# reazon-research/ReazonSpeech

Measured on AMD Instinct MI355X. Metric: RTFx (audio-sec/wall-sec), FastConformer-RNNT 619M batch=256, higher is better.
Workload: dtype bf16

## Files before the change

reazonspeech_amd/csrc/k_rnnt.hip:

```cpp
#include <cstdio>
#include <cstdlib>

#include "k_rnnt_common.h"

namespace {

__global__ void rnnt_init_kernel(DecodeState st, const int32_t* __restrict__ enc_lens, int B, int blank,
                                 int32_t* __restrict__ n_ids) {
    __shared__ int n_alive_s;
    if (threadIdx.x == 0) n_alive_s = 0;
    __syncthreads();
    for (int b = threadIdx.x; b < B; b += blockDim.x) {
        st.tcur[b] = 0; st.sym[b] = 0; st.token[b] = blank; st.act[b] = b;
        if (st.token2) st.token2[b] = -1;
        n_ids[b] = 0;
        if (enc_lens[b] > 0) st.alive[atomicAdd(&n_alive_s, 1)] = b;
    }
    __syncthreads();
    if (threadIdx.x == 0) { st.counters[0] = B; st.counters[1] = 0; st.counters[2] = n_alive_s; st.counters[3] = 0; }
}

__global__ __launch_bounds__(1024) void rnnt_lstm_kernel(DecodeState st, int layer, int B, int H,
                                                        const float* __restrict__ embed,
                                                        const float* __restrict__ W ,
                                                        const float* __restrict__ bias ) {
    extern __shared__ __attribute__((aligned(16))) char lstm_smem[];
    float (*part)[4][32][16] = reinterpret_cast<float (*)[4][32][16]>(lstm_smem);
    int* rows_s = reinterpret_cast<int*>(lstm_smem + SPLITK_LSTM * 4 * 32 * 16 * 4);
    const int n_act = st.counters[0];
    const int rt = blockIdx.y, ut = blockIdx.x;
    if (rt * 32 >= n_act) return;
    const int tid = threadIdx.x, lane = tid & 63, wave = tid >> 6;
    if (tid < 32) {
        const int i = rt * 32 + tid;
        rows_s[tid] = st.act[i < n_act ? i : n_act - 1];
    }
    __syncthreads();
    const int li = lane & 15, kk = lane >> 4;
    const int lr = lane >> 2, lc = lane & 3;
    const int perm = 4 * (4 * li + kk);
    const int K = 2 * H, kslice = K / SPLITK_LSTM, nkb = K / 16;
    const float* xsrc[2];
    const float* hsrc[2];
#pragma unroll
    for (int ri = 0; ri < 2; ++ri) {
        const int row = rows_s[ri * 16 + lr];
        xsrc[ri] = layer == 0 ? embed + (size_t)st.token[row] * H : st.h_tmp + ((size_t)(layer - 1) * B + row) * H;
        hsrc[ri] = st.h + ((size_t)layer * B + row) * H;
    }
    const float* wfrag[4];
#pragma unroll
    for (int gt = 0; gt < 4; ++gt) wfrag[gt] = W + ((size_t)((gt * H) / 16 + ut) * nkb) * 256 + lane * 4;
    f32x4_t acc[2][4];
#pragma unroll
    for (int ri = 0; ri < 2; ++ri)
#pragma unroll
        for (int gt = 0; gt < 4; ++gt) acc[ri][gt] = (f32x4_t){0.f, 0.f, 0.f, 0.f};
    struct Frag { float4 a[2], w[4]; };
    auto load = [&](int k0) {
        Frag fr;
        const int k = k0 + 4 * lc;
#pragma unroll
        for (int ri = 0; ri < 2; ++ri)
            fr.a[ri] = (k < H) ? *reinterpret_cast<const float4*>(xsrc[ri] + k)
                               : *reinterpret_cast<const float4*>(hsrc[ri] + (k - H));
#pragma unroll
        for (int gt = 0; gt < 4; ++gt) fr.w[gt] = *reinterpret_cast<const float4*>(wfrag[gt] + (size_t)(k0 >> 4) * 256);
        return fr;
    };
    auto compute = [&](const Frag& fin) {
        Frag fr = fin;
#pragma unroll
        for (int ri = 0; ri < 2; ++ri) fr.a[ri] = to_mfma_a_layout(fin.a[ri], perm);
#define RS_MFMA_E(c)                                                                                            \
        _Pragma("unroll") for (int ri = 0; ri < 2; ++ri) _Pragma("unroll") for (int gt = 0; gt < 4; ++gt)      \
            acc[ri][gt] = __builtin_amdgcn_mfma_f32_16x16x4f32(fr.a[ri].c, fr.w[gt].c, acc[ri][gt], 0, 0, 0);
        RS_MFMA_E(x) RS_MFMA_E(y) RS_MFMA_E(z) RS_MFMA_E(w)
#undef RS_MFMA_E
    };
    const int kbeg = wave * kslice, nblk = kslice / 16;
    {
        Frag f0 = load(kbeg);
        Frag f1 = nblk > 1 ? load(kbeg + 16) : f0;
        int u = 0;
        for (; u + 2 < nblk; ++u) {
            const Frag f2 = load(kbeg + 16 * (u + 2));
            compute(f0);
            f0 = f1;
            f1 = f2;
        }
        if (nblk >= 2) { compute(f0); f0 = f1; }
        compute(f0);
    }
#pragma unroll
    for (int ri = 0; ri < 2; ++ri)
#pragma unroll
        for (int gt = 0; gt < 4; ++gt)
#pragma unroll
            for (int r = 0; r < 4; ++r) part[wave][gt][ri * 16 + 4 * kk + r][li] = acc[ri][gt][r];
    __syncthreads();
    if (tid >= 512) return;
    const int i = tid >> 4, j = tid & 15;
    if (rt * 32 + i >= n_act) return;
    const int brow = rows_s[i];
    const int unit = ut * 16 + j;
    float z[4];
#pragma unroll
    for (int gt = 0; gt < 4; ++gt) {
        float s = part[0][gt][i][j];
#pragma unroll
        for (int sl = 1; sl < SPLITK_LSTM; ++sl) s = s + part[sl][gt][i][j];
        z[gt] = s + bias[gt * H + unit];
    }
    const float ig = rs_sigmoidf(z[0]), fg = rs_sigmoidf(z[1]), gg = rs_tanhf(z[2]), og = rs_sigmoidf(z[3]);
    const size_t o = ((size_t)layer * B + brow) * H + unit;
    const float cn = fmaf(fg, st.c[o], ig * gg);
    st.c_tmp[o] = cn;
    st.h_tmp[o] = og * rs_tanhf(cn);
}

template <int MODE>
__global__ __launch_bounds__(512) void rnnt_tile_kernel(DecodeState st, const float* __restrict__ f, int B, int Tp,
                                                        int L, int H, int K, int N, const float* __restrict__ W,
                                                        const float* __restrict__ bias, int n_ctiles, int step,
                                                        int rows_per_utt) {
    extern __shared__ __attribute__((aligned(16))) char tile_smem[];
    float (*part)[32][65] = reinterpret_cast<float (*)[32][65]>(tile_smem);
    int* rows_s = reinterpret_cast<int*>(tile_smem + SPLITK_TILE * 32 * 65 * 4);
    int rt = blockIdx.y;
    const int ct = blockIdx.x;
    const int tid = threadIdx.x, lane = tid & 63, wave = tid >> 6;
    constexpr bool WALK = MODE == 3 || MODE == 4;
    constexpr bool ARGMAX = MODE == 1 || MODE == 5;
    const int32_t* list = MODE == 0 ? st.act : st.alive + (size_t)(step & 1) * B;
    const int la = MODE == 5 ? rows_per_utt : 1;
    const int n_rows = MODE == 0 ? st.counters[0] : st.counters[2 + (step & 1)] * la;
    if (MODE >= 1 && rt == 0 && ct == 0 && tid == 0) {
        st.counters[0] = 0;
        st.counters[2 + ((step + 1) & 1)] = 0;
    }
    if (MODE >= 1 && ct >= n_ctiles) return;
    for (;; rt += gridDim.y) {
    if (rt * 32 >= n_rows) return;
    if (tid < 32) {
        int i = rt * 32 + tid;
        i = i < n_rows ? i : n_rows - 1;
        rows_s[tid] = MODE == 5 ? list[i / la] * la + i % la : list[i];
    }
    __syncthreads();
    const int li = lane & 15, kk = lane >> 4;
    const int lr = lane >> 2, lc = lane & 3;
    const int perm = 4 * (4 * li + kk);
    const float* asrc[2];
    const float* gsrc[2];
#pragma unroll
    for (int ri = 0; ri < 2; ++ri) {
        const int row = rows_s[ri * 16 + lr];
        if (MODE == 0) {
            asrc[ri] = st.h_tmp + ((size_t)(L - 1) * B + row) * H;
            gsrc[ri] = nullptr;
        } else {
            if (MODE == 4) {
                asrc[ri] = st.a_pre + (size_t)row * K;
                gsrc[ri] = nullptr;
            } else if (MODE == 5) {
                const int utt = row / la;
                int t = st.tcur[utt] + row % la;
                t = t < Tp ? t : Tp - 1;
                asrc[ri] = f + ((size_t)utt * Tp + t) * K;
                gsrc[ri] = st.g + (size_t)utt * K;
            } else {
                int t = st.tcur[row];
                t = t < Tp ? t : Tp - 1;
                const int utt = MODE >= 2 ? row / rows_per_utt : row;
                asrc[ri] = f + ((size_t)utt * Tp + t) * K;
                gsrc[ri] = MODE == 3 ? st.g + st.g_off[row] : st.g + (size_t)row * K;
            }
        }
    }
    const int nkb = K / 16, ntile = (N + 15) / 16;
    const float* wfrag[4];
#pragma unroll
    for (int cj = 0; cj < 4; ++cj) {
        int tn = ct * 4 + cj;
        tn = tn < ntile ? tn : ntile - 1;
        wfrag[cj] = W + ((size_t)tn * nkb) * 256 + lane * 4;
    }
    f32x4_t acc[2][4];
#pragma unroll
    for (int ri = 0; ri < 2; ++ri)
#pragma unroll
        for (int cj = 0; cj < 4; ++cj) acc[ri][cj] = (f32x4_t){0.f, 0.f, 0.f, 0.f};
    constexpr bool HAS_G = (MODE >= 1 && MODE <= 3) || MODE == 5;
    struct Frag { float4 a[2], g[2], w[4]; };
    auto load = [&](int k0) {
        Frag fr;
        const int k = k0 + 4 * lc;
#pragma unroll
        for (int ri = 0; ri < 2; ++ri) {
            fr.a[ri] = *reinterpret_cast<const float4*>(asrc[ri] + k);
            if (HAS_G) fr.g[ri] = *reinterpret_cast<const float4*>(gsrc[ri] + k);
        }
#pragma unroll
        for (int cj = 0; cj < 4; ++cj) fr.w[cj] = *reinterpret_cast<const float4*>(wfrag[cj] + (size_t)(k0 >> 4) * 256);
        return fr;
    };
    auto compute = [&](const Frag& fr) {
        float4 a[2];
#pragma unroll
        for (int ri = 0; ri < 2; ++ri) {
            a[ri] = fr.a[ri];
            if (HAS_G) {
                if (st.joint_act) {
                    a[ri].x = rs_tanhf(a[ri].x + fr.g[ri].x); a[ri].y = rs_tanhf(a[ri].y + fr.g[ri].y);
                    a[ri].z = rs_tanhf(a[ri].z + fr.g[ri].z); a[ri].w = rs_tanhf(a[ri].w + fr.g[ri].w);
// ... 94 lines not shown
        const int oi = st.pidx[(size_t)b * n_ctiles + ctile];
        if (ov > val || (ov == val && oi < idx)) { val = ov; idx = oi; }
    }
#pragma unroll
    for (int off = 32; off > 0; off >>= 1) {
        const float ov = __shfl_xor(val, off, 64);
        const int oi = __shfl_xor(idx, off, 64);
        if (ov > val || (ov == val && oi < idx)) { val = ov; idx = oi; }
    }
    if (lane != 0) return;
    int t = st.tcur[b], sy = st.sym[b];
    bool emitted = false;
    if (idx == blank || idx == st.unk || idx == 0x7fffffff) {
        t += 1; sy = 0;
    } else {
        const int n = n_ids[b];
        if (n < u_max) { ids[(size_t)b * u_max + n] = idx; frames[(size_t)b * u_max + n] = t; n_ids[b] = n + 1; }
        else st.counters[1] = 1;
        if (st.token2) st.token2[b] = st.token[b];
        st.token[b] = idx;
        emitted = true;
        sy += 1;
        if (sy >= max_symbols) { t += 1; sy = 0; }
    }
    st.tcur[b] = t; st.sym[b] = sy;
    if (t < enc_lens[b]) {
        const int pos = atomicAdd(&st.counters[2 + ((step + 1) & 1)], 1);
        st.alive[(size_t)((step + 1) & 1) * B + pos] = b;
        if (emitted) { const int pa = atomicAdd(&st.counters[0], 1); st.act[pa] = b; }
    }
}



__global__ __launch_bounds__(256) void rnnt_finalize_la_kernel(DecodeState st, const int32_t* __restrict__ enc_lens, int B, int n_ctiles,
                                                               int blank, int max_symbols, int u_max, int step, int la,
                                                               int32_t* __restrict__ ids, int32_t* __restrict__ frames,
                                                               int32_t* __restrict__ n_ids) {
    const int lane = threadIdx.x & 63;
    const int slot = blockIdx.x * 4 + (threadIdx.x >> 6);
    const int n_alive = st.counters[2 + (step & 1)];
    if (slot >= n_alive) return;
    const int b = st.alive[(size_t)(step & 1) * B + slot];
    const int T = enc_lens[b];
    int t = st.tcur[b], sy = st.sym[b];
    bool emitted = false;
    for (int j = 0; j < la && t < T; ++j) {
        float val = -INFINITY;
        int idx = 0x7fffffff;
        const size_t row = (size_t)b * la + j;
        for (int ctile = lane; ctile < n_ctiles; ctile += 64) {
            const float ov = st.pmax[row * n_ctiles + ctile];
            const int oi = st.pidx[row * n_ctiles + ctile];
            if (ov > val || (ov == val && oi < idx)) { val = ov; idx = oi; }
        }
#pragma unroll
        for (int off = 32; off > 0; off >>= 1) {
            const float ov = __shfl_xor(val, off, 64);
            const int oi = __shfl_xor(idx, off, 64);
            if (ov > val || (ov == val && oi < idx)) { val = ov; idx = oi; }
        }
        if (idx == blank || idx == st.unk || idx == 0x7fffffff) { t += 1; sy = 0; continue; }
        if (lane == 0) {
            const int n = n_ids[b];
            if (n < u_max) { ids[(size_t)b * u_max + n] = idx; frames[(size_t)b * u_max + n] = t; n_ids[b] = n + 1; }
            else st.counters[1] = 1;
            if (st.token2) st.token2[b] = st.token[b];
            st.token[b] = idx;
        }
        emitted = true;
        sy += 1;
        if (sy >= max_symbols) { t += 1; sy = 0; }
        break;
    }
    if (lane != 0) return;
    st.tcur[b] = t; st.sym[b] = sy;
    if (t < T) {
        const int pos = atomicAdd(&st.counters[2 + ((step + 1) & 1)], 1);
        st.alive[(size_t)((step + 1) & 1) * B + pos] = b;
        if (emitted) { const int pa = atomicAdd(&st.counters[0], 1); st.act[pa] = b; }
    }
}

__global__ __launch_bounds__(1024) void rnnt_lstm4_kernel(DecodeState st, int layer, int B, int H,
                                                         const float* __restrict__ embed,
                                                         const float* __restrict__ W4 ,
                                                         const float* __restrict__ bias ) {
    __shared__ float part[SPLITK_LSTM][32][17];
    __shared__ int rows_s[32];
    const int n_act = st.counters[0];
    const int rt = blockIdx.y, ug = blockIdx.x;
    if (rt * 32 >= n_act) return;
    const int tid = threadIdx.x, lane = tid & 63, wave = tid >> 6;
    if (tid < 32) {
        const int i = rt * 32 + tid;
        rows_s[tid] = st.act[i < n_act ? i : n_act - 1];
    }
    __syncthreads();
    const int li = lane & 15, kk = lane >> 4;
    const int lr = lane >> 2, lc = lane & 3;
    const int perm = 4 * (4 * li + kk);
    const int K = 2 * H, kslice = K / SPLITK_LSTM, nkb = K / 16;
    const float* xsrc[2];
    const float* hsrc[2];
#pragma unroll
    for (int ri = 0; ri < 2; ++ri) {
        const int row = rows_s[ri * 16 + lr];
        xsrc[ri] = layer == 0 ? embed + (size_t)st.token[row] * H : st.h_tmp + ((size_t)(layer - 1) * B + row) * H;
        hsrc[ri] = st.h + ((size_t)layer * B + row) * H;
    }
    const float* wfrag = W4 + ((size_t)ug * nkb) * 256 + lane * 4;
    f32x4_t acc[2] = {(f32x4_t){0.f, 0.f, 0.f, 0.f}, (f32x4_t){0.f, 0.f, 0.f, 0.f}};
    const int kbeg = wave * kslice, nblk = kslice / 16;
    float4 av[2][8], wv[8];
#pragma unroll
    for (int u = 0; u < 8; ++u)
        if (u < nblk) {
            const int k = kbeg + 16 * u + 4 * lc;
#pragma unroll
            for (int ri = 0; ri < 2; ++ri)
                av[ri][u] = (k < H) ? *reinterpret_cast<const float4*>(xsrc[ri] + k) : *reinterpret_cast<const float4*>(hsrc[ri] + (k - H));
            wv[u] = *reinterpret_cast<const float4*>(wfrag + (size_t)((kbeg >> 4) + u) * 256);
        }
#pragma unroll
    for (int u = 0; u < 8; ++u)
        if (u < nblk) {
            const float4 a0 = to_mfma_a_layout(av[0][u], perm), a1 = to_mfma_a_layout(av[1][u], perm);
#define RS_MFMA_E(c)                                                                         \
            acc[0] = __builtin_amdgcn_mfma_f32_16x16x4f32(a0.c, wv[u].c, acc[0], 0, 0, 0);   \
            acc[1] = __builtin_amdgcn_mfma_f32_16x16x4f32(a1.c, wv[u].c, acc[1], 0, 0, 0);
            RS_MFMA_E(x) RS_MFMA_E(y) RS_MFMA_E(z) RS_MFMA_E(w)
#undef RS_MFMA_E
        }
#pragma unroll
    for (int ri = 0; ri < 2; ++ri)
#pragma unroll
        for (int r = 0; r < 4; ++r) part[wave][ri * 16 + 4 * kk + r][li] = acc[ri][r];
    __syncthreads();
    if (tid >= 128) return;
    const int i = tid >> 2, u4 = tid & 3;
    if (rt * 32 + i >= n_act) return;
    const int brow = rows_s[i];
    const int unit = ug * 4 + u4;
    float z[4];
#pragma unroll
    for (int gt = 0; gt < 4; ++gt) {
        float sm = part[0][i][gt * 4 + u4];
#pragma unroll
        for (int sl = 1; sl < SPLITK_LSTM; ++sl) sm = sm + part[sl][i][gt * 4 + u4];
        z[gt] = sm + bias[gt * H + unit];
    }
    const float ig = rs_sigmoidf(z[0]), fg = rs_sigmoidf(z[1]), gg = rs_tanhf(z[2]), og = rs_sigmoidf(z[3]);
    const size_t o = ((size_t)layer * B + brow) * H + unit;
    const float cn = fmaf(fg, st.c[o], ig * gg);
    st.c_tmp[o] = cn;
    st.h_tmp[o] = og * rs_tanhf(cn);
}

__global__ __launch_bounds__(512) void rnnt_pred16_kernel(DecodeState st, int B, int L, int H, int N ,
                                                         const float* __restrict__ W, const float* __restrict__ bias) {
    __shared__ float part[SPLITK_TILE][32][17];
    __shared__ int rows_s[32];
    const int rt = blockIdx.y, ct = blockIdx.x;
    const int tid = threadIdx.x, lane = tid & 63, wave = tid >> 6;
    const int n_rows = st.counters[0];
    if (rt * 32 >= n_rows) return;
    if (tid < 32) {
        const int i = rt * 32 + tid;
        rows_s[tid] = st.act[i < n_rows ? i : n_rows - 1];
    }
    __syncthreads();
    const int li = lane & 15, kk = lane >> 4;
    const int lr = lane >> 2, lc = lane & 3;
    const int perm = 4 * (4 * li + kk);
    const int K = H, nkb = K / 16;
    const float* asrc[2];
#pragma unroll
    for (int ri = 0; ri < 2; ++ri) asrc[ri] = st.h_tmp + ((size_t)(L - 1) * B + rows_s[ri * 16 + lr]) * H;
    const float* wfrag = W + ((size_t)ct * nkb) * 256 + lane * 4;
    f32x4_t acc[2] = {(f32x4_t){0.f, 0.f, 0.f, 0.f}, (f32x4_t){0.f, 0.f, 0.f, 0.f}};
    const int kslice = K / SPLITK_TILE, kbeg = wave * kslice, nblk = kslice / 16;
    float4 av[2][8], wv[8];
#pragma unroll
    for (int u = 0; u < 8; ++u)
        if (u < nblk) {
            const int k = kbeg + 16 * u + 4 * lc;
#pragma unroll
            for (int ri = 0; ri < 2; ++ri) av[ri][u] = *reinterpret_cast<const float4*>(asrc[ri] + k);
            wv[u] = *reinterpret_cast<const float4*>(wfrag + (size_t)((kbeg >> 4) + u) * 256);
        }
#pragma unroll
    for (int u = 0; u < 8; ++u)
        if (u < nblk) {
            const float4 a0 = to_mfma_a_layout(av[0][u], perm), a1 = to_mfma_a_layout(av[1][u], perm);
#define RS_MFMA_E(c)                                                                         \
            acc[0] = __builtin_amdgcn_mfma_f32_16x16x4f32(a0.c, wv[u].c, acc[0], 0, 0, 0);   \
            acc[1] = __builtin_amdgcn_mfma_f32_16x16x4f32(a1.c, wv[u].c, acc[1], 0, 0, 0);
            RS_MFMA_E(x) RS_MFMA_E(y) RS_MFMA_E(z) RS_MFMA_E(w)
#undef RS_MFMA_E
        }
#pragma unroll
    for (int ri = 0; ri < 2; ++ri)
#pragma unroll
        for (int r = 0; r < 4; ++r) part[wave][ri * 16 + 4 * kk + r][li] = acc[ri][r];
    __syncthreads();
    const int i = tid >> 4, c = tid & 15;
    const bool row_ok = rt * 32 + i < n_rows;
    const int brow = rows_s[i];
    const int v = ct * 16 + c;
    if (row_ok && v < N) {
        float sm = part[0][i][c];
#pragma unroll
        for (int sl = 1; sl < SPLITK_TILE; ++sl) sm = sm + part[sl][i][c];
        st.g[(size_t)brow * N + v] = sm + bias[v];
    }
    if (row_ok) {
        const int nct = gridDim.x;
        for (int l = 0; l < L; ++l)
            for (int u = ct * 16 + c; u < H; u += nct * 16) {
                const size_t o = ((size_t)l * B + brow) * H + u;
                st.h[o] = st.h_tmp[o];
                st.c[o] = st.c_tmp[o];
            }
    }
}

__global__ __launch_bounds__(256) void rnnt_prep_kernel(DecodeState st, const float* __restrict__ f, int B, int Tp, int J,
                                                        int step) {
    const int lane = threadIdx.x & 63;
    const int slot = blockIdx.x * 4 + (threadIdx.x >> 6);
    if (blockIdx.x == 0 && threadIdx.x == 0) {
        st.counters[0] = 0;
        st.counters[2 + ((step + 1) & 1)] = 0;
    }
    if (slot >= st.counters[2 + (step & 1)]) return;
    const int b = st.alive[(size_t)(step & 1) * B + slot];
    int t = st.tcur[b];
    t = t < Tp ? t : Tp - 1;
    const float* fr = f + ((size_t)b * Tp + t) * J;
    const float* gr = st.g + (size_t)b * J;
    float ss = 0.0f;
    for (int k = 4 * lane; k < J; k += 256) {
        const float4 fv = *reinterpret_cast<const float4*>(fr + k), gv = *reinterpret_cast<const float4*>(gr + k);
        float a0, a1, a2, a3;
        if (st.joint_act) {
            a0 = rs_tanhf(fv.x + gv.x); a1 = rs_tanhf(fv.y + gv.y); a2 = rs_tanhf(fv.z + gv.z); a3 = rs_tanhf(fv.w + gv.w);
        } else {
            a0 = fmaxf(fv.x + gv.x, 0.0f); a1 = fmaxf(fv.y + gv.y, 0.0f); a2 = fmaxf(fv.z + gv.z, 0.0f); a3 = fmaxf(fv.w + gv.w, 0.0f);
        }
        ss = fmaf(a0, a0, fmaf(a1, a1, fmaf(a2, a2, fmaf(a3, a3, ss))));
        *reinterpret_cast<u16x4_t*>(st.a16 + (size_t)slot * J + k) = pack_bf16x4(a0, a1, a2, a3);
    }
    ss = wave_sum(ss);
    if (lane == 0) st.anorm[slot] = sqrtf(ss) * 1.0001f + 0x1p-55f;
}

__global__ __launch_bounds__(256) void rnnt_screen_kernel(DecodeState st, const float* __restrict__ f, int B, int Tp, int J,
                                                          int Vpad, const uint16_t* __restrict__ W16,
                                                          const float* __restrict__ bpad, int step) {
    extern __shared__ __attribute__((aligned(16))) char scr_smem[];
    const int ldrow = J * 2 + 16;
    const int ct = blockIdx.x, rt = blockIdx.y;
    const int tid = threadIdx.x, lane = tid & 63, wave = tid >> 6;
    const int n_alive = st.counters[2 + (step & 1)];
    if (rt * 32 >= n_alive) return;
    const int col0 = (ct * 4 + wave) * 16;
    const bool has_cols = col0 < Vpad;
    const int li = lane & 15, kc = lane >> 4;
    const int nks = J / 32;
    const uint16_t* wrow = W16 + (size_t)((has_cols ? col0 : 0) + li) * J + kc * 8;
    bf16x8_t wf[20];
#pragma unroll
    for (int q = 0; q < 20; ++q)
        if (q < nks) wf[q] = *reinterpret_cast<const bf16x8_t*>(wrow + q * 32);
    const float bv = bpad[(has_cols ? col0 : 0) + li];
    {
        const int per_row = J / 8;
        for (int idx = tid; idx < 32 * per_row; idx += 256) {
            const int r = idx / per_row, c = idx - r * per_row;
            const int i = rt * 32 + r;
            const uint4 v = *reinterpret_cast<const uint4*>(st.a16 + (size_t)(i < n_alive ? i : n_alive - 1) * J + c * 8);
            *reinterpret_cast<uint4*>(scr_smem + r * ldrow + c * 16) = v;
        }
    }
    __syncthreads();
    if (!has_cols) return;
    f32x4_t acc[2] = {(f32x4_t){0.f, 0.f, 0.f, 0.f}, (f32x4_t){0.f, 0.f, 0.f, 0.f}};
#pragma unroll
    for (int q = 0; q < 20; ++q)
        if (q < nks) {
#pragma unroll
            for (int ri = 0; ri < 2; ++ri) {
                const bf16x8_t af = *reinterpret_cast<const bf16x8_t*>(scr_smem + (ri * 16 + li) * ldrow + (q * 32 + kc * 8) * 2);
                acc[ri] = __builtin_amdgcn_mfma_f32_16x16x32_bf16(af, wf[q], acc[ri], 0, 0, 0);
            }
        }
#pragma unroll
    for (int ri = 0; ri < 2; ++ri)
#pragma unroll
        for (int r = 0; r < 4; ++r) {
            const int slot = rt * 32 + ri * 16 + 4 * kc + r;
            if (slot < n_alive) st.zapprox[(size_t)slot * Vpad + col0 + li] = acc[ri][r] + bv;
        }
}

__device__ __forceinline__ float screen_margin(float m, float wmax, float anorm) {
// ... 167 lines not shown
    float zr[NCHW];
#pragma unroll
    for (int c = 0; c < NCHW; ++c) {
        const int col = (wave * NCHW + c) * 64 + lane;
        zr[c] = col < V ? z[col] : -INFINITY;
    }
    float m = -INFINITY;
#pragma unroll
    for (int c = 0; c < NCHW; ++c) m = fmaxf(m, zr[c]);
    m = wave_max(m);
    float* a_s = reinterpret_cast<float*>(ver_smem);
    int* cand_s = reinterpret_cast<int*>(ver_smem + (size_t)J * 4) + wave * (NCHW * 64);
    float* red = reinterpret_cast<float*>(ver_smem + (size_t)J * 4 + (size_t)4 * NCHW * 64 * 4);
    const int t = st.tcur[b];
    const int tc = t < Tp ? t : Tp - 1;
    verify_act_row(st, f + ((size_t)b * Tp + tc) * J, st.g + (size_t)b * J, a_s, J, threadIdx.x, 256);
    if (lane == 0) red[wave] = m;
    __syncthreads();
    m = fmaxf(fmaxf(red[0], red[1]), fmaxf(red[2], red[3]));
    const float margin = screen_margin(m, wmax[0], st.anorm[slot]);
    int n_cand = 0;
#pragma unroll
    for (int c = 0; c < NCHW; ++c) {
        const bool is = screen_candidate(m, zr[c], margin);
        const unsigned long long mask = __ballot(is);
        if (is) cand_s[n_cand + __builtin_popcountll(mask & ((1ull << lane) - 1ull))] = (wave * NCHW + c) * 64 + lane;
        n_cand += __builtin_popcountll(mask);
    }
    __builtin_amdgcn_fence(__ATOMIC_ACQ_REL, "wavefront");
    __builtin_amdgcn_wave_barrier();
    float best = -INFINITY;
    int best_idx = 0x7fffffff;
    verify_evaluate(cand_s, n_cand, a_s, Wrm, bo, J, lane, best, best_idx);
    if (lane == 0) { red[4 + wave] = best; reinterpret_cast<int*>(red)[8 + wave] = best_idx; }
    __syncthreads();
    if (threadIdx.x != 0) return;
#pragma unroll
    for (int w = 0; w < 4; ++w) {
        const float v = red[4 + w];
        const int i = reinterpret_cast<int*>(red)[8 + w];
        if (v > best || (v == best && i < best_idx)) { best = v; best_idx = i; }
    }
    verify_commit(st, b, t, best_idx, enc_lens, B, blank, max_symbols, u_max, step, ids, frames, n_ids);
}

}


namespace {

__global__ __launch_bounds__(256) void k2_decoder_kernel(DecodeState st, int B, int D, const float* __restrict__ embed,
                                                         const float* __restrict__ conv_w ) {
    const int n_rows = st.counters[0];
    if ((int)blockIdx.x >= n_rows) return;
    const int row = st.act[blockIdx.x];
    const int t0 = st.token2[row], t1 = st.token[row];
    for (int c = threadIdx.x; c < D; c += 256) {
        const int g4 = c & ~3;
        float acc = 0.0f;
#pragma unroll
        for (int i = 0; i < 4; ++i) {
            const float e = t0 >= 0 ? embed[(size_t)t0 * D + g4 + i] : 0.0f;
            acc = fmaf(conv_w[(c * 4 + i) * 2 + 0], e, acc);
        }
#pragma unroll
        for (int i = 0; i < 4; ++i) {
            const float e = t1 >= 0 ? embed[(size_t)t1 * D + g4 + i] : 0.0f;
            acc = fmaf(conv_w[(c * 4 + i) * 2 + 1], e, acc);
        }
        st.h_tmp[(size_t)row * D + c] = fmaxf(acc, 0.0f);
    }
}

constexpr int LSTM_LDS = SPLITK_LSTM * 4 * 32 * 16 * 4 + 32 * 4;
constexpr int TILE_LDS = SPLITK_TILE * 32 * 65 * 4 + 32 * 4;

bool narrow_kernels_usable(const rs_ctx* ctx) {
    const int L = ctx->d.pred_layers, H = ctx->d.pred_hidden;
    bool narrow = ctx->decode_narrow;
    for (int l = 0; l < L; ++l) narrow = narrow && ctx->lstm_w4[l] != nullptr;
    return narrow && 2 * H / SPLITK_LSTM / 16 <= 8 && H / SPLITK_TILE / 16 <= 8;
}

void launch_lstm_pred(rs_ctx* ctx, const DecodeState& st, int B, int rows_bound, bool narrow, hipStream_t s) {
    const int L = ctx->d.pred_layers, H = ctx->d.pred_hidden, J = ctx->d.joint_hidden;
    const int rts = (rows_bound + 31) / 32 > 0 ? (rows_bound + 31) / 32 : 1;
    if (ctx->k2_conv_w) {
        hipLaunchKernelGGL(k2_decoder_kernel, dim3(rows_bound > 0 ? rows_bound : 1), dim3(256), 0, s, st, B, H, ctx->embed, ctx->k2_conv_w);
        hipLaunchKernelGGL(rnnt_pred16_kernel, dim3((J + 15) / 16, rts), dim3(512), 0, s, st, B, 1, H, J, ctx->jpred_w, ctx->jpred_b);
        return;
    }
    if (narrow) {
        for (int l = 0; l < L; ++l)
            hipLaunchKernelGGL(rnnt_lstm4_kernel, dim3(H / 4, rts), dim3(1024), 0, s, st, l, B, H, ctx->embed, ctx->lstm_w4[l],
                               ctx->lstm_b[l]);
        hipLaunchKernelGGL(rnnt_pred16_kernel, dim3((J + 15) / 16, rts), dim3(512), 0, s, st, B, L, H, J, ctx->jpred_w,
                           ctx->jpred_b);
        return;
    }
    for (int l = 0; l < L; ++l)
        hipLaunchKernelGGL(rnnt_lstm_kernel, dim3(H / 16, rts), dim3(1024), LSTM_LDS, s, st, l, B, H, ctx->embed,
                           ctx->lstm_w[l], ctx->lstm_b[l]);
    hipLaunchKernelGGL(rnnt_tile_kernel<0>, dim3((J + 63) / 64, rts), dim3(512), TILE_LDS, s, st, (const float*)nullptr, B,
                       0, L, H, H, J, ctx->jpred_w, ctx->jpred_b, 0, 0, 1);
}

int joint_grid_x(int nct, int rts) {
    return rts > 1 && !rs_knob(RS_KNOB_DECODE_NO_XCD) ? (nct + 7) / 8 * 8 : nct;
}

int ensure_decode_lds(rs_ctx* ctx) {
    if (int rc = rs_ensure_dynamic_lds(ctx, (const void*)rnnt_lstm_kernel, LSTM_LDS); rc != RS_OK) return rc;
    if (int rc = rs_ensure_dynamic_lds(ctx, (const void*)rnnt_tile_kernel<0>, TILE_LDS); rc != RS_OK) return rc;
    if (int rc = rs_ensure_dynamic_lds(ctx, (const void*)rnnt_tile_kernel<1>, TILE_LDS); rc != RS_OK) return rc;
    if (int rc = rs_ensure_dynamic_lds(ctx, (const void*)rnnt_tile_kernel<2>, TILE_LDS); rc != RS_OK) return rc;
    if (int rc = rs_ensure_dynamic_lds(ctx, (const void*)rnnt_tile_kernel<3>, TILE_LDS); rc != RS_OK) return rc;
    if (int rc = rs_ensure_dynamic_lds(ctx, (const void*)rnnt_tile_kernel<4>, TILE_LDS); rc != RS_OK) return rc;
    return rs_ensure_dynamic_lds(ctx, (const void*)rnnt_tile_kernel<5>, TILE_LDS);
}

}

int rs_rnnt_launch_lstm_pred(rs_ctx* ctx, const void* st_ptr, int rows, hipStream_t s) {
    if (int rc = ensure_decode_lds(ctx); rc != RS_OK) return rc;
    launch_lstm_pred(ctx, *reinterpret_cast<const DecodeState*>(st_ptr), rows, rows, narrow_kernels_usable(ctx), s);
    return RS_OK;
}

int rs_rnnt_launch_joint_logits(rs_ctx* ctx, const void* st_ptr, const float* joint_enc, int rows, int tp_max, int rows_per_utt,
                                int step, hipStream_t s) {
    if (int rc = ensure_decode_lds(ctx); rc != RS_OK) return rc;
    const rs_dims& d = ctx->d;
    const int nct = rs_joint_zstride(d) / 64;
    hipLaunchKernelGGL(rnnt_tile_kernel<2>, dim3(joint_grid_x(nct, (rows + 31) / 32), (rows + 31) / 32), dim3(512), TILE_LDS, s,
                       *reinterpret_cast<const DecodeState*>(st_ptr), joint_enc, rows, tp_max, d.pred_layers, d.pred_hidden,
                       d.joint_hidden, d.n_logits, ctx->jout_w, ctx->jout_b, nct, step, rows_per_utt);
    return RS_OK;
}

int rs_rnnt_launch_joint_logits_indirect(rs_ctx* ctx, const void* st_ptr, const float* joint_enc, int rows, int rows_bound, int tp_max,
                                         int rows_per_utt, int step, hipStream_t s) {
    if (int rc = ensure_decode_lds(ctx); rc != RS_OK) return rc;
    const rs_dims& d = ctx->d;
    const int nct = rs_joint_zstride(d) / 64;
    const int rts = (rows_bound + 31) / 32 > 0 ? (rows_bound + 31) / 32 : 1;
    const DecodeState& st = *reinterpret_cast<const DecodeState*>(st_ptr);
    if (st.a_pre)
        hipLaunchKernelGGL(rnnt_tile_kernel<4>, dim3(joint_grid_x(nct, rts), rts), dim3(512), TILE_LDS, s, st, joint_enc, rows, tp_max,
                           d.pred_layers, d.pred_hidden, d.joint_hidden, d.n_logits, ctx->jout_w, ctx->jout_b, nct, step, rows_per_utt);
    else
        hipLaunchKernelGGL(rnnt_tile_kernel<3>, dim3(joint_grid_x(nct, rts), rts), dim3(512), TILE_LDS, s, st, joint_enc, rows, tp_max,
                           d.pred_layers, d.pred_hidden, d.joint_hidden, d.n_logits, ctx->jout_w, ctx->jout_b, nct, step, rows_per_utt);
    return RS_OK;
}

constexpr int LOOKAHEAD_MAX = 8;

static void greedy_layout(const rs_ctx* ctx, int B, rs_arena& a, DecodeState& st) {
    const rs_dims& d = ctx->d;
    const size_t state = (size_t)d.pred_layers * B * d.pred_hidden, J = d.joint_hidden;
    const size_t nct = (d.n_logits + 63) / 64, Vpad = (size_t)(d.n_logits + 15) / 16 * 16;
    st.h = a.take<float>(state); st.c = a.take<float>(state);
    st.h_tmp = a.take<float>(state); st.c_tmp = a.take<float>(state);
    st.g = a.take<float>(B * J);
    st.tcur = a.take<int32_t>(B); st.sym = a.take<int32_t>(B);
    st.token = a.take<int32_t>(B); st.act = a.take<int32_t>(B);
    if (ctx->k2_conv_w) st.token2 = a.take<int32_t>(B);
    st.alive = a.take<int32_t>((size_t)2 * B);
    st.counters = a.take<int32_t>(16);
    st.pmax = a.take<float>(B * LOOKAHEAD_MAX * nct); st.pidx = a.take<int32_t>(B * LOOKAHEAD_MAX * nct);
    st.a16 = a.take<uint16_t>(B * J); st.anorm = a.take<float>(B);
    st.zapprox = a.take<float>(B * Vpad);
}

size_t rs_rnnt_workspace_bytes(const rs_ctx* ctx, int B) {
    rs_arena a;
    DecodeState st{};
    greedy_layout(ctx, B, a, st);
    return a.bytes() + RS_DECODE_SLACK;
}

int rs_rnnt_greedy_impl(rs_ctx* ctx, const float* joint_enc, const int32_t* enc_lens, int B, int tp_max, int u_max,
                        int32_t* ids, int32_t* frames, int32_t* n_ids, void* workspace, size_t workspace_bytes,
                        hipStream_t s) {
    const rs_dims& d = ctx->d;
    const int L = d.pred_layers, H = d.pred_hidden, J = d.joint_hidden, V = d.n_logits;
    if (B <= 0) return RS_OK;
    if (int rc = rs_rnnt_check_dims(ctx, "rnnt"); rc != RS_OK) return rc;
    rs_arena arena(workspace);
    DecodeState st{};
    greedy_layout(ctx, B, arena, st);
    if (workspace_bytes < arena.bytes() + RS_DECODE_SLACK) return rs_fail(ctx, RS_EWORKSPACE, "rnnt: workspace too small");
    st.joint_act = d.joint_act;
    if (ctx->k2_conv_w) st.unk = rs_k2_unk_id(ctx);
    const size_t state_bytes = (size_t)L * B * H * 4;
    const int nct = (V + 63) / 64, Vpad = (V + 15) / 16 * 16;
    const bool screen = ctx->decode_screen && ctx->jout_w16 && ctx->jout_wrm && ctx->jout_bpad && ctx->jout_wmax &&
                        J / SPLITK_TILE / 16 <= 8 && J / 32 <= 20;

    if (int rc = ensure_decode_lds(ctx); rc != RS_OK) return rc;
    const bool narrow = narrow_kernels_usable(ctx);
    auto lstm_and_pred = [&](int rows_bound) { launch_lstm_pred(ctx, st, B, rows_bound, narrow, s); };

    rs_prof_scope prof(ctx, RS_PROF_DECODE, s, 0.0, 0.0);
    RS_HIP(ctx, hipMemsetAsync(st.h, 0, 2 * rs_align(state_bytes), s));
    RS_HIP(ctx, hipMemsetAsync(st.g, 0, (size_t)B * J * 4, s));
    hipLaunchKernelGGL(rnnt_init_kernel, dim3(1), dim3(256), 0, s, st, enc_lens, B, d.blank_id, n_ids);
    lstm_and_pred(B);
    RS_CHECK_LAUNCH(ctx, "rnnt init");

    const int max_steps = tp_max + (u_max < tp_max * d.max_symbols ? u_max : tp_max * d.max_symbols) + 1;
    const int CHUNK = 16;
    const bool lookahead = !rs_knob(RS_KNOB_DECODE_NO_LOOKAHEAD);
    const bool verify_wide = rs_knob(RS_KNOB_VERIFY_WIDE) != 0;
    int32_t host_counters[4] = {0, 0, 0, 0};
    int steps = 0, alive_bound = B;
    bool finished = false;
    while (!finished && steps < max_steps) {
        for (int c = 0; c < CHUNK; ++c, ++steps) {
            const int rows = alive_bound < B ? alive_bound : B;
            if (screen) {
                const int rts = (rows + 31) / 32 > 0 ? (rows + 31) / 32 : 1;
                hipLaunchKernelGGL(rnnt_prep_kernel, dim3((rows + 3) / 4 > 0 ? (rows + 3) / 4 : 1), dim3(256), 0, s, st, joint_enc, B,
                                   tp_max, J, steps);
                hipLaunchKernelGGL(rnnt_screen_kernel, dim3((Vpad + 63) / 64, rts), dim3(256), 32 * (J * 2 + 16), s, st, joint_enc, B,
                                   tp_max, J, Vpad, ctx->jout_w16, ctx->jout_bpad, steps);
                const dim3 vg((rows + 3) / 4 > 0 ? (rows + 3) / 4 : 1), vgw(rows > 0 ? rows : 1);
#define RS_VERIFY_ARGS st, joint_enc, enc_lens, B, tp_max, J, V, Vpad, ctx->jout_wrm, ctx->jout_b, ctx->jout_wmax, d.blank_id, d.max_symbols, u_max, steps, ids, frames, n_ids
                if (V > 64 * 48 && V <= 4 * 64 * 48)
                    hipLaunchKernelGGL(rnnt_verify_wide_kernel<48>, vgw, dim3(256), J * 4 + 4 * 48 * 64 * 4 + 64, s, RS_VERIFY_ARGS);
                else if (V > 64 * 48)
                    hipLaunchKernelGGL(rnnt_verify_kernel<0>, vg, dim3(256), 4 * J * 4 + 4 * VER_CAP * 4, s, RS_VERIFY_ARGS);
                else if (verify_wide)
                    hipLaunchKernelGGL(rnnt_verify_wide_kernel<12>, vgw, dim3(256), J * 4 + 4 * 12 * 64 * 4 + 64, s, RS_VERIFY_ARGS);
                else if (V <= 64 * 8)
                    hipLaunchKernelGGL(rnnt_verify_kernel<8>, vg, dim3(256), 4 * J * 4 + 4 * 8 * 64 * 4, s, RS_VERIFY_ARGS);
                else
                    hipLaunchKernelGGL(rnnt_verify_kernel<48>, vg, dim3(256), 4 * J * 4 + 4 * 48 * 64 * 4, s, RS_VERIFY_ARGS);
#undef RS_VERIFY_ARGS
            } else {
                int la = 1;
                if (lookahead) while (la < LOOKAHEAD_MAX && 2 * la * (rows > 0 ? rows : 1) <= 256) la *= 2;
                if (la > 1) {
                    const int rts = (rows * la + 31) / 32 > 0 ? (rows * la + 31) / 32 : 1;
                    hipLaunchKernelGGL(rnnt_tile_kernel<5>, dim3(joint_grid_x(nct, rts), rts), dim3(512), TILE_LDS, s, st, joint_enc, B, tp_max, L, H,
                                       J, V, ctx->jout_w, ctx->jout_b, nct, steps, la);
                    hipLaunchKernelGGL(rnnt_finalize_la_kernel, dim3((rows + 3) / 4 > 0 ? (rows + 3) / 4 : 1), dim3(256), 0, s, st, enc_lens, B, nct,
                                       d.blank_id, d.max_symbols, u_max, steps, la, ids, frames, n_ids);
                } else {
                    const int rts = (rows + 31) / 32 > 0 ? (rows + 31) / 32 : 1;
                    hipLaunchKernelGGL(rnnt_tile_kernel<1>, dim3(joint_grid_x(nct, rts), rts), dim3(512), TILE_LDS, s, st, joint_enc, B, tp_max, L, H,
                                       J, V, ctx->jout_w, ctx->jout_b, nct, steps, 1);
                    hipLaunchKernelGGL(rnnt_finalize_kernel, dim3((rows + 3) / 4 > 0 ? (rows + 3) / 4 : 1), dim3(256), 0, s, st, enc_lens, B, nct,
                                       d.blank_id, d.max_symbols, u_max, steps, ids, frames, n_ids);
                }
            }
            lstm_and_pred(rows);
        }
        RS_CHECK_LAUNCH(ctx, "rnnt step");
        RS_HIP(ctx, hipMemcpyAsync(host_counters, st.counters, 4 * sizeof(int32_t), hipMemcpyDeviceToHost, s));
        RS_HIP(ctx, hipStreamSynchronize(s));
        finished = host_counters[2 + (steps & 1)] == 0;
        alive_bound = host_counters[2 + (steps & 1)];
    }
    prof.end();
    if (rs_knob(RS_KNOB_DECODE_TRACE)) fprintf(stderr, "[decode trace] B=%d T'=%d: %d steps (screen %d, narrow %d, lookahead %d)\n", B, tp_max, steps, (int)screen, (int)narrow, (int)lookahead);
    if (host_counters[1]) return rs_fail(ctx, RS_EOVERFLOW, "rnnt: an utterance emitted more than u_max=%d tokens", u_max);
    if (!finished) return rs_fail(ctx, RS_ESTATE, "rnnt: decode did not finish in %d steps", max_steps);
    return RS_OK;
}
```

reazonspeech_amd/csrc/rs_knobs.h:

```cpp
#pragma once
#include <stdlib.h>
#include <string.h>

#include <atomic>
#include <mutex>

#include "../../include/rs_asr.h"

#define RS_KNOBS(X)                                                                                                                   \
    X(GEMM_TILE, "RS_GEMM_TILE", INT, 0, "forced GEMM tile height (256 / 192 / 128 / 64); 0 = by shape")                              \
    X(GEMM_GROUP_M, "RS_GEMM_GROUP_M", INT, 0, "row panels per XCD tile group; 0 = by shape")                                         \
    X(GEMM_PAIRS, "RS_GEMM_PAIRS", INT, 2, "2 = two tiles per workgroup, LDS ring carried over; 1 = ring restarted; 0 = one tile")    \
    X(GEMM_BREG, "RS_GEMM_BREG", INT, 0, "1 = 256- / 192-row launches keep the weight operand out of LDS (global -> VGPR)")           \
    X(ATTN_PERSIST, "RS_ATTN_PERSIST", INT, 0, "1 = full attention on resident workgroups that walk the items (n >= 2: on n)")        \
    X(ATTN_STREAM, "RS_ATTN_STREAM", INT, 0, "1 = the streaming attention form (+ 16 x mask: phases left out, for timing)")           \
    X(ATTN64, "RS_ATTN64", INT, 4, "head_dim 64: key blocks per chunk; 0 = the one-workgroup-per-CU geometry")                        \
    X(ATTN64_NW, "RS_ATTN64_NW", INT, 4, "head_dim 64: waves per workgroup (the second number of $RS_ATTN64)")                        \
    X(ATTN_F32_OLD, "RS_ATTN_F32_OLD", PRESENT, 0, "float32 attention: the first form (one wave per key sum)")                        \
    X(ATTN_F32_KEYS, "RS_ATTN_F32_KEYS", PRESENT, 0, "float32 attention: the second form (keys over lanes, no MFMA)")                 \
    X(GLU_GENERIC, "RS_GLU_GENERIC", INT, 0, "GLU + depthwise conv: 1 = the any-kernel-size path, 2 = the f32-tile kernel on the gated layout") \
    X(SUB_IM2COL, "RS_SUB_IM2COL", PRESENT, 0, "ESPnet subsampling: gather the 3 x 3 patches into a matrix first (sizes the workspace too)") \
    X(FUSE_GLU, "RS_FUSE_GLU", INT, 1, "context default: 0 = GLU in the depthwise kernel, not the pw1 GEMM epilogue")                 \
    X(DEFER_OUT_NORM, "RS_DEFER_OUT_NORM", INT, 1, "context default: 0 = every output norm stores its f32 rows")                      \
    X(DECODE_SCREEN, "RS_DECODE_SCREEN", INT, 1, "context default: 0 = exact evaluation of every joint column")                       \
    X(DECODE_NARROW, "RS_DECODE_NARROW", INT, 1, "context default: 0 = the wide-tile LSTM / projection kernels")                      \
    X(DECODE_NO_XCD, "RS_DECODE_NO_XCD", PRESENT, 0, "greedy decode: joint grids not padded to a multiple of 8 column tiles")         \
    X(DECODE_NO_LOOKAHEAD, "RS_DECODE_NO_LOOKAHEAD", PRESENT, 0, "greedy decode: one frame per utterance and step at every batch size") \
    X(VERIFY_WIDE, "RS_VERIFY_WIDE", INT, 0, "screened joint: 1 = a workgroup per row for V <= 3072 too")                             \
    X(DECODE_TRACE, "RS_DECODE_TRACE", PRESENT, 0, "greedy decode: print the step count of every call to stderr")                     \
    X(BEAM_SPEC, "RS_BEAM_SPEC", INT, 3, "beam search: evaluations asked for per iteration (1 .. 8; sizes the workspace too)")         \
    X(BEAM_TRACE, "RS_BEAM_TRACE", PRESENT, 0, "beam search: phase timing of the step kernel")                                        \
    X(BEAM_RECORD_LDS, "RS_BEAM_RECORD_LDS", PRESENT, 0, "beam search: the any-vocabulary record kernel on a small vocabulary")       \
    X(AVSR_POSCONV_OLD, "RS_AVSR_POSCONV_OLD", PRESENT, 0, "AV-HuBERT positional convolution: the VALU form")                         \
    X(K2_CONV1_OLD, "RS_K2_CONV1_OLD", PRESENT, 0, "Zipformer conv1: the VALU form (the one other channel counts run)")               \
    X(K2_ATTW_SWEEPS, "RS_K2_ATTW_SWEEPS", INT, 1, "Zipformer attention weights: 3 = the three-sweep kernel")                         \
    X(K2_CONV2_FUSED, "RS_K2_CONV2_FUSED", INT, 1, "default of option k2_conv2_fused: 0 = patch matrix + GEMM launch")                \
    X(K2_CNX_FUSED, "RS_K2_CNX_FUSED", INT, 1, "default of option k2_cnx_fused: 0 = the ConvNeXt pointwise pair as two GEMM launches")

enum rs_knob_id {
#define RS_KNOB_ENUM(id, env, kind, def, what) RS_KNOB_##id,
    RS_KNOBS(RS_KNOB_ENUM)
#undef RS_KNOB_ENUM
    RS_KNOB_COUNT
};
enum rs_knob_kind { RS_KNOB_PRESENT, RS_KNOB_INT };
struct rs_knob_row { const char* env; rs_knob_kind kind; int def; };
static const rs_knob_row rs_knob_rows[RS_KNOB_COUNT] = {
#define RS_KNOB_ROW(id, env, kind, def, what) {env, RS_KNOB_##kind, def},
    RS_KNOBS(RS_KNOB_ROW)
#undef RS_KNOB_ROW
};

struct rs_knob_table {
    std::atomic<int> value[RS_KNOB_COUNT];
    std::atomic<bool> given[RS_KNOB_COUNT];
    std::once_flag once;
};
inline rs_knob_table rs_knob_state;

inline void rs_knobs_read_env() {
    std::call_once(rs_knob_state.once, [] {
        rs_knob_table& t = rs_knob_state;
        for (int i = 0; i < RS_KNOB_COUNT; ++i) { t.value[i] = rs_knob_rows[i].def; t.given[i] = false; }
        for (int i = 0; i < RS_KNOB_COUNT; ++i) {
            const char* e = i == RS_KNOB_ATTN64_NW ? nullptr : getenv(rs_knob_rows[i].env);
            if (!e) continue;
            t.given[i] = true;
            t.value[i] = rs_knob_rows[i].kind == RS_KNOB_PRESENT ? 1 : atoi(e);
            if (i == RS_KNOB_ATTN64) {
                t.given[RS_KNOB_ATTN64_NW] = true;
                if (const char* c = strchr(e, ',')) t.value[RS_KNOB_ATTN64_NW] = atoi(c + 1);
            }
        }
    });
}

inline int rs_knob(rs_knob_id id) { rs_knobs_read_env(); return rs_knob_state.value[id].load(std::memory_order_relaxed); }
inline bool rs_knob_given(rs_knob_id id) { rs_knobs_read_env(); return rs_knob_state.given[id].load(std::memory_order_relaxed); }
inline void rs_knob_set(rs_knob_id id, int v) { rs_knobs_read_env(); rs_knob_state.value[id].store(v, std::memory_order_relaxed); }

inline int rs_knob_find(const char* env_name) {
    for (int i = 0; env_name && i < RS_KNOB_COUNT; ++i)
        if (!strcmp(env_name, rs_knob_rows[i].env)) return i;
    return -1;
}
inline int rs_knob_set_named(const char* env_name, int v) {
    const int i = rs_knob_find(env_name);
    if (i < 0) return RS_EINVAL;
    rs_knob_set((rs_knob_id)i, v);
    return RS_OK;
}
inline int rs_knob_get_named(const char* env_name, int* v) {
    const int i = rs_knob_find(env_name);
    if (i < 0 || !v) return RS_EINVAL;
    *v = rs_knob((rs_knob_id)i);
    return RS_OK;
}
```

Measured before the change: 46190.

## Let LSTM/projection workgroups walk row tiles and keep weight fragments in registers

The narrow LSTM and prediction-projection kernels become templated on the per-wave block count and loop over row tiles with a grid stride. Weight fragments are loaded once on the first tile and kept in registers for the following tiles. A new knob, RS_DECODE_ROWWALK, caps the row-tile grid dimension, but it defaults to 0, which keeps one workgroup per 32 rows, so by default each workgroup still handles a single tile. Any default gain would come from the NBLK templating, which removes the runtime guards. The wide LSTM kernel and tile MODE 0 also gain the walking form.

```diff
diff --git a/reazonspeech_amd/csrc/k_rnnt.hip b/reazonspeech_amd/csrc/k_rnnt.hip
--- a/reazonspeech_amd/csrc/k_rnnt.hip
+++ b/reazonspeech_amd/csrc/k_rnnt.hip
@@ -28,18 +28,19 @@
     float (*part)[4][32][16] = reinterpret_cast<float (*)[4][32][16]>(lstm_smem);
     int* rows_s = reinterpret_cast<int*>(lstm_smem + SPLITK_LSTM * 4 * 32 * 16 * 4);
     const int n_act = st.counters[0];
-    const int rt = blockIdx.y, ut = blockIdx.x;
-    if (rt * 32 >= n_act) return;
-    const int tid = threadIdx.x, lane = tid & 63, wave = tid >> 6;
+    const int K = 2 * H, kslice = K / SPLITK_LSTM, nkb = K / 16;
+    for (int rt = blockIdx.y; rt * 32 < n_act; rt += gridDim.y) {
+    int tid = threadIdx.x, ut = blockIdx.x;
+    asm volatile("" : "+v"(tid), "+s"(ut));
+    const int lane = tid & 63, wave = __builtin_amdgcn_readfirstlane(tid >> 6);
+    const int li = lane & 15, kk = lane >> 4;
+    const int lr = lane >> 2, lc = lane & 3;
+    const int perm = 4 * (4 * li + kk);
     if (tid < 32) {
         const int i = rt * 32 + tid;
         rows_s[tid] = st.act[i < n_act ? i : n_act - 1];
     }
     __syncthreads();
-    const int li = lane & 15, kk = lane >> 4;
-    const int lr = lane >> 2, lc = lane & 3;
-    const int perm = 4 * (4 * li + kk);
-    const int K = 2 * H, kslice = K / SPLITK_LSTM, nkb = K / 16;
     const float* xsrc[2];
     const float* hsrc[2];
 #pragma unroll
@@ -99,9 +100,8 @@
 #pragma unroll
             for (int r = 0; r < 4; ++r) part[wave][gt][ri * 16 + 4 * kk + r][li] = acc[ri][gt][r];
     __syncthreads();
-    if (tid >= 512) return;
     const int i = tid >> 4, j = tid & 15;
-    if (rt * 32 + i >= n_act) return;
+    if (tid < 512 && rt * 32 + i < n_act) {
     const int brow = rows_s[i];
     const int unit = ut * 16 + j;
     float z[4];
@@ -117,6 +117,9 @@
     const float cn = fmaf(fg, st.c[o], ig * gg);
     st.c_tmp[o] = cn;
     st.h_tmp[o] = og * rs_tanhf(cn);
+    }
+    __syncthreads();
+    }
 }
 
 template <int MODE>
@@ -130,7 +133,7 @@
     int rt = blockIdx.y;
     const int ct = blockIdx.x;
     const int tid = threadIdx.x, lane = tid & 63, wave = tid >> 6;
-    constexpr bool WALK = MODE == 3 || MODE == 4;
+    constexpr bool WALK = MODE == 0 || MODE == 3 || MODE == 4;
     constexpr bool ARGMAX = MODE == 1 || MODE == 5;
     const int32_t* list = MODE == 0 ? st.act : st.alive + (size_t)(step & 1) * B;
     const int la = MODE == 5 ? rows_per_utt : 1;
@@ -391,6 +394,7 @@
     }
 }
 
+template <int NBLK>
 __global__ __launch_bounds__(1024) void rnnt_lstm4_kernel(DecodeState st, int layer, int B, int H,
                                                          const float* __restrict__ embed,
                                                          const float* __restrict__ W4 ,
@@ -398,18 +402,26 @@
     __shared__ float part[SPLITK_LSTM][32][17];
     __shared__ int rows_s[32];
     const int n_act = st.counters[0];
-    const int rt = blockIdx.y, ug = blockIdx.x;
-    if (rt * 32 >= n_act) return;
-    const int tid = threadIdx.x, lane = tid & 63, wave = tid >> 6;
+    const int ug = blockIdx.x;
+    if ((int)blockIdx.y * 32 >= n_act) return;
+    const int wave = threadIdx.x >> 6;
+    const int K = 2 * H, kslice = K / SPLITK_LSTM, nkb = K / 16;
+    const float* wfrag = W4 + ((size_t)ug * nkb) * 256 + (threadIdx.x & 63) * 4;
+    const int kbeg = wave * kslice;
+    float4 wv[NBLK];
+    for (int rt = blockIdx.y; rt * 32 < n_act; rt += gridDim.y) {
+    int tid = threadIdx.x;
+    asm volatile("" : "+v"(tid));
+    const int lane = tid & 63;
+    const int li = lane & 15, kk = lane >> 4;
+    const int lr = lane >> 2, lc = lane & 3;
+    const int perm = 4 * (4 * li + kk);
     if (tid < 32) {
         const int i = rt * 32 + tid;
         rows_s[tid] = st.act[i < n_act ? i : n_act - 1];
     }
     __syncthreads();
-    const int li = lane & 15, kk = lane >> 4;
-    const int lr = lane >> 2, lc = lane & 3;
-    const int perm = 4 * (4 * li + kk);
-    const int K = 2 * H, kslice = K / SPLITK_LSTM, nkb = K / 16;
+    float4 av[2][NBLK];
     const float* xsrc[2];
     const float* hsrc[2];
 #pragma unroll
@@ -418,22 +430,17 @@
         xsrc[ri] = layer == 0 ? embed + (size_t)st.token[row] * H : st.h_tmp + ((size_t)(layer - 1) * B + row) * H;
         hsrc[ri] = st.h + ((size_t)layer * B + row) * H;
     }
-    const float* wfrag = W4 + ((size_t)ug * nkb) * 256 + lane * 4;
     f32x4_t acc[2] = {(f32x4_t){0.f, 0.f, 0.f, 0.f}, (f32x4_t){0.f, 0.f, 0.f, 0.f}};
-    const int kbeg = wave * kslice, nblk = kslice / 16;
-    float4 av[2][8], wv[8];
-#pragma unroll
-    for (int u = 0; u < 8; ++u)
-        if (u < nblk) {
+#pragma unroll
+    for (int u = 0; u < NBLK; ++u) {
             const int k = kbeg + 16 * u + 4 * lc;
 #pragma unroll
             for (int ri = 0; ri < 2; ++ri)
                 av[ri][u] = (k < H) ? *reinterpret_cast<const float4*>(xsrc[ri] + k) : *reinterpret_cast<const float4*>(hsrc[ri] + (k - H));
-            wv[u] = *reinterpret_cast<const float4*>(wfrag + (size_t)((kbeg >> 4) + u) * 256);
-        }
-#pragma unroll
-    for (int u = 0; u < 8; ++u)
-        if (u < nblk) {
+            if (rt == (int)blockIdx.y) wv[u] = *reinterpret_cast<const float4*>(wfrag + (size_t)((kbeg >> 4) + u) * 256);
+        }
+#pragma unroll
+    for (int u = 0; u < NBLK; ++u) {
             const float4 a0 = to_mfma_a_layout(av[0][u], perm), a1 = to_mfma_a_layout(av[1][u], perm);
 #define RS_MFMA_E(c)                                                                         \
             acc[0] = __builtin_amdgcn_mfma_f32_16x16x4f32(a0.c, wv[u].c, acc[0], 0, 0, 0);   \
@@ -446,9 +453,8 @@
 #pragma unroll
         for (int r = 0; r < 4; ++r) part[wave][ri * 16 + 4 * kk + r][li] = acc[ri][r];
     __syncthreads();
-    if (tid >= 128) return;
     const int i = tid >> 2, u4 = tid & 3;
-    if (rt * 32 + i >= n_act) return;
+    if (tid < 128 && rt * 32 + i < n_act) {
     const int brow = rows_s[i];
     const int unit = ug * 4 + u4;
     float z[4];
@@ -464,43 +470,50 @@
     const float cn = fmaf(fg, st.c[o], ig * gg);
     st.c_tmp[o] = cn;
     st.h_tmp[o] = og * rs_tanhf(cn);
-}
-
+    }
+    if ((rt + (int)gridDim.y) * 32 < n_act) __syncthreads();
+    }
+}
+
+template <int NBLK>
 __global__ __launch_bounds__(512) void rnnt_pred16_kernel(DecodeState st, int B, int L, int H, int N ,
                                                          const float* __restrict__ W, const float* __restrict__ bias) {
     __shared__ float part[SPLITK_TILE][32][17];
     __shared__ int rows_s[32];
-    const int rt = blockIdx.y, ct = blockIdx.x;
-    const int tid = threadIdx.x, lane = tid & 63, wave = tid >> 6;
+    const int ct = blockIdx.x;
+    const int wave = threadIdx.x >> 6;
     const int n_rows = st.counters[0];
-    if (rt * 32 >= n_rows) return;
+    if ((int)blockIdx.y * 32 >= n_rows) return;
+    const int K = H, nkb = K / 16;
+    const float* wfrag = W + ((size_t)ct * nkb) * 256 + (threadIdx.x & 63) * 4;
+    const int kslice = K / SPLITK_TILE, kbeg = wave * kslice;
+    float4 wv[NBLK];
+    for (int rt = blockIdx.y; rt * 32 < n_rows; rt += gridDim.y) {
+    int tid = threadIdx.x;
+    asm volatile("" : "+v"(tid));
+    const int lane = tid & 63;
+    const int li = lane & 15, kk = lane >> 4;
+    const int lr = lane >> 2, lc = lane & 3;
+    const int perm = 4 * (4 * li + kk);
     if (tid < 32) {
         const int i = rt * 32 + tid;
         rows_s[tid] = st.act[i < n_rows ? i : n_rows - 1];
     }
     __syncthreads();
-    const int li = lane & 15, kk = lane >> 4;
-    const int lr = lane >> 2, lc = lane & 3;
-    const int perm = 4 * (4 * li + kk);
-    const int K = H, nkb = K / 16;
+    float4 av[2][NBLK];
     const float* asrc[2];
 #pragma unroll
     for (int ri = 0; ri < 2; ++ri) asrc[ri] = st.h_tmp + ((size_t)(L - 1) * B + rows_s[ri * 16 + lr]) * H;
-    const float* wfrag = W + ((size_t)ct * nkb) * 256 + lane * 4;
     f32x4_t acc[2] = {(f32x4_t){0.f, 0.f, 0.f, 0.f}, (f32x4_t){0.f, 0.f, 0.f, 0.f}};
-    const int kslice = K / SPLITK_TILE, kbeg = wave * kslice, nblk = kslice / 16;
-    float4 av[2][8], wv[8];
-#pragma unroll
-    for (int u = 0; u < 8; ++u)
-        if (u < nblk) {
+#pragma unroll
+    for (int u = 0; u < NBLK; ++u) {
             const int k = kbeg + 16 * u + 4 * lc;
 #pragma unroll
             for (int ri = 0; ri < 2; ++ri) av[ri][u] = *reinterpret_cast<const float4*>(asrc[ri] + k);
-            wv[u] = *reinterpret_cast<const float4*>(wfrag + (size_t)((kbeg >> 4) + u) * 256);
-        }
-#pragma unroll
-    for (int u = 0; u < 8; ++u)
-        if (u < nblk) {
+            if (rt == (int)blockIdx.y) wv[u] = *reinterpret_cast<const float4*>(wfrag + (size_t)((kbeg >> 4) + u) * 256);
+        }
+#pragma unroll
+    for (int u = 0; u < NBLK; ++u) {
             const float4 a0 = to_mfma_a_layout(av[0][u], perm), a1 = to_mfma_a_layout(av[1][u], perm);
 #define RS_MFMA_E(c)                                                                         \
             acc[0] = __builtin_amdgcn_mfma_f32_16x16x4f32(a0.c, wv[u].c, acc[0], 0, 0, 0);   \
@@ -531,6 +544,8 @@
                 st.h[o] = st.h_tmp[o];
                 st.c[o] = st.c_tmp[o];
             }
+    }
+    if ((rt + (int)gridDim.y) * 32 < n_rows) __syncthreads();
     }
 }
 
@@ -864,20 +879,35 @@
     return narrow && 2 * H / SPLITK_LSTM / 16 <= 8 && H / SPLITK_TILE / 16 <= 8;
 }
 
-void launch_lstm_pred(rs_ctx* ctx, const DecodeState& st, int B, int rows_bound, bool narrow, hipStream_t s) {
+#define RS_NBLK_SWITCH(H, LAUNCH)                                                                       \
+    switch ((H) / 128) {                                                                                \
+        case 1: LAUNCH(1); break; case 2: LAUNCH(2); break; case 3: LAUNCH(3); break; case 4: LAUNCH(4); break; \
+        case 5: LAUNCH(5); break; case 6: LAUNCH(6); break; case 7: LAUNCH(7); break; default: LAUNCH(8); break; \
+    }
+void launch_lstm4(dim3 grid, hipStream_t s, const DecodeState& st, int layer, int B, int H, const float* embed, const float* W4,
+                  const float* bias) {
+#define RS_LAUNCH(N) hipLaunchKernelGGL(rnnt_lstm4_kernel<N>, grid, dim3(1024), 0, s, st, layer, B, H, embed, W4, bias)
+    RS_NBLK_SWITCH(H, RS_LAUNCH)
+#undef RS_LAUNCH
+}
+void launch_pred16(dim3 grid, hipStream_t s, const DecodeState& st, int B, int L, int H, int N, const float* W, const float* bias) {
+#define RS_LAUNCH(N_) hipLaunchKernelGGL(rnnt_pred16_kernel<N_>, grid, dim3(512), 0, s, st, B, L, H, N, W, bias)
+    RS_NBLK_SWITCH(H, RS_LAUNCH)
+#undef RS_LAUNCH
+}
+#undef RS_NBLK_SWITCH
+
+void launch_lstm_pred(rs_ctx* ctx, const DecodeState& st, int B, int rows_bound, int row_extent, bool narrow, hipStream_t s) {
     const int L = ctx->d.pred_layers, H = ctx->d.pred_hidden, J = ctx->d.joint_hidden;
-    const int rts = (rows_bound + 31) / 32 > 0 ? (rows_bound + 31) / 32 : 1;
+    const int rts = row_extent > 0 ? row_extent : 1;
     if (ctx->k2_conv_w) {
         hipLaunchKernelGGL(k2_decoder_kernel, dim3(rows_bound > 0 ? rows_bound : 1), dim3(256), 0, s, st, B, H, ctx->embed, ctx->k2_conv_w);
-        hipLaunchKernelGGL(rnnt_pred16_kernel, dim3((J + 15) / 16, rts), dim3(512), 0, s, st, B, 1, H, J, ctx->jpred_w, ctx->jpred_b);
+        launch_pred16(dim3((J + 15) / 16, rts), s, st, B, 1, H, J, ctx->jpred_w, ctx->jpred_b);
         return;
     }
     if (narrow) {
-        for (int l = 0; l < L; ++l)
-            hipLaunchKernelGGL(rnnt_lstm4_kernel, dim3(H / 4, rts), dim3(1024), 0, s, st, l, B, H, ctx->embed, ctx->lstm_w4[l],
-                               ctx->lstm_b[l]);
-        hipLaunchKernelGGL(rnnt_pred16_kernel, dim3((J + 15) / 16, rts), dim3(512), 0, s, st, B, L, H, J, ctx->jpred_w,
-                           ctx->jpred_b);
+        for (int l = 0; l < L; ++l) launch_lstm4(dim3(H / 4, rts), s, st, l, B, H, ctx->embed, ctx->lstm_w4[l], ctx->lstm_b[l]);
+        launch_pred16(dim3((J + 15) / 16, rts), s, st, B, L, H, J, ctx->jpred_w, ctx->jpred_b);
         return;
     }
     for (int l = 0; l < L; ++l)
@@ -905,7 +935,7 @@
 
 int rs_rnnt_launch_lstm_pred(rs_ctx* ctx, const void* st_ptr, int rows, hipStream_t s) {
     if (int rc = ensure_decode_lds(ctx); rc != RS_OK) return rc;
-    launch_lstm_pred(ctx, *reinterpret_cast<const DecodeState*>(st_ptr), rows, rows, narrow_kernels_usable(ctx), s);
+    launch_lstm_pred(ctx, *reinterpret_cast<const DecodeState*>(st_ptr), rows, rows, (rows + 31) / 32, narrow_kernels_usable(ctx), s);
     return RS_OK;
 }
 
@@ -982,7 +1012,11 @@
 
     if (int rc = ensure_decode_lds(ctx); rc != RS_OK) return rc;
     const bool narrow = narrow_kernels_usable(ctx);
-    auto lstm_and_pred = [&](int rows_bound) { launch_lstm_pred(ctx, st, B, rows_bound, narrow, s); };
+    const int rowwalk = rs_knob(RS_KNOB_DECODE_ROWWALK);
+    auto lstm_and_pred = [&](int rows_bound) {
+        const int rts = (rows_bound + 31) / 32;
+        launch_lstm_pred(ctx, st, B, rows_bound, rowwalk > 0 && rowwalk < rts ? rowwalk : rts, narrow, s);
+    };
 
     rs_prof_scope prof(ctx, RS_PROF_DECODE, s, 0.0, 0.0);
     RS_HIP(ctx, hipMemsetAsync(st.h, 0, 2 * rs_align(state_bytes), s));
diff --git a/reazonspeech_amd/csrc/rs_knobs.h b/reazonspeech_amd/csrc/rs_knobs.h
--- a/reazonspeech_amd/csrc/rs_knobs.h
+++ b/reazonspeech_amd/csrc/rs_knobs.h
@@ -24,6 +24,7 @@
     X(DEFER_OUT_NORM, "RS_DEFER_OUT_NORM", INT, 1, "context default: 0 = every output norm stores its f32 rows")                      \
     X(DECODE_SCREEN, "RS_DECODE_SCREEN", INT, 1, "context default: 0 = exact evaluation of every joint column")                       \
     X(DECODE_NARROW, "RS_DECODE_NARROW", INT, 1, "context default: 0 = the wide-tile LSTM / projection kernels")                      \
+    X(DECODE_ROWWALK, "RS_DECODE_ROWWALK", INT, 0, "greedy decode: n > 0 = at most n LSTM / projection workgroups per column slice, walking the row tiles; 0 = one per 32 alive rows") \
     X(DECODE_NO_XCD, "RS_DECODE_NO_XCD", PRESENT, 0, "greedy decode: joint grids not padded to a multiple of 8 column tiles")         \
     X(DECODE_NO_LOOKAHEAD, "RS_DECODE_NO_LOOKAHEAD", PRESENT, 0, "greedy decode: one frame per utterance and step at every batch size") \
     X(VERIFY_WIDE, "RS_VERIFY_WIDE", INT, 0, "screened joint: 1 = a workgroup per row for V <= 3072 too")                             \
```

Result: no change. 46240, median of 2 (+0.1%).
